# noisystreet/aither

Hardware: AMD Instinct MI355X
Metric: Mcell-updates/sec per iteration (residual+LU-SGS), 256^3 block; % HBM roofline (higher is better)
Workload: dtype f64

## Files before the change

### aither_amd/csrc/agx_api.hip

```cpp
#include "agx_kernels.hpp"
#include "agx_geometry.hpp"
#include "agx_mem.hpp"
#include "agx_switches.hpp"
#include <rccl/rccl.h>
#include <cstdarg>
#include <cstdio>
#include <cstring>
#include <cstdlib>
#include <cmath>
#include <vector>
#include <array>
#include <map>
#include <string>
#include <algorithm>
#include <memory>
#include <type_traits>

using namespace agx;

static char g_err[512] = "";
static int fail(const char* fmt, ...) {
  va_list ap;
  va_start(ap, fmt);
  vsnprintf(g_err, sizeof g_err, fmt, ap);
// ... 14 lines not shown
auto by_bool(bool v, F f) {
  return v ? f(std::true_type{}) : f(std::false_type{});
}
template <int V0, int... Vs, class F>
auto by_int(int v, F f) {
  if constexpr (sizeof...(Vs) == 0) return f(std::integral_constant<int, V0>{});
  else return v == V0 ? f(std::integral_constant<int, V0>{}) : by_int<Vs...>(v, f);
}

struct SweepGraphs {
  hipGraphExec_t g[2][2][2] = {};
  SweepGraphs() = default;
  SweepGraphs(SweepGraphs&& o) noexcept { memcpy(g, o.g, sizeof g); memset(o.g, 0, sizeof g); }
  ~SweepGraphs() { drop(); }
  hipGraphExec_t& at(bool forward, bool full, bool un_is_u) { return g[forward][full][un_is_u]; }
  void drop() {
    for (auto& g1 : g) for (auto& g2 : g1) for (auto& g3 : g2)
      if (g3) { hipGraphExecDestroy(g3); g3 = nullptr; }
  }
};

struct Block {
  BlockDev d;
  int global_pos = 0;
  DevBuf<double> slab;
  DevBuf<double> d2;
  DevBuf<double> blockmat;
  DevBuf<double> sweep_rec;
  bool sweep_geo_built = false;
  bool x_planes_current = false;
  bool x_is_zero = false;
  bool d2_state_current = false;
  bool resid_norms_current = false;
  DevBuf<double> mg_forcing, mg_mres, mg_xsave, mg_nodes;
  DevBuf<int> mg_tc, mg_start;
  DevBuf<double> mg_vf, mg_cf;
  const void *mg_tc_key = nullptr, *mg_vf_key = nullptr, *mg_cf_key = nullptr;
  bool node_built = false;
  DevBuf<double> nodes_dev, fcen;
  DevBuf<int> d2_tab;
  std::vector<int> dstart;
  SweepGraphs sweep_graph;
  DevBuf<int> kp_mem;
  unsigned kp_epoch = 0;
  long d2idx(int i, int j, int k) const {
    const int ie = i + d.ng, je = j + d.ng, de = ie + je;
    return (long)(k + d.ng) * d.d2.ps + dstart[de] + je - std::max(0, de - (d.d2.Pi - 1));
  }
  bool state_is_a = true;
  DevBuf<agx_bc_surface> surf_dev;
  std::vector<agx_bc_surface> surf_host;
  DevBuf<int> nr_off_dev;
  DevBuf<double> nr_mem;
  long nr_max = 0;
  DevBuf<int> wall_off_dev;
  DevBuf<WallVars> wall_mem;
  std::vector<WallSurfDev> wall_tab;
  DevBuf<WallSurfDev> wall_tab_dev;
  long wall_faces = 0;
  std::vector<LoadSurfDev> load_tab;
  DevBuf<LoadSurfDev> load_tab_dev;
  long load_faces = 0, load_chunks = 0;
  DevBuf<double> load_partial, load_fcen;
};

struct ConnSide {
// ... 94 lines not shown
  std::vector<std::pair<hipEvent_t, hipEvent_t>> ev_pool;
  std::vector<std::pair<int, int>> ev_used;
  double t_ms[G_NGROUP] = {};
  long t_n[G_NGROUP] = {};
};

static int my_side(const agx_ctx* c, const Conn& k);
static int implicit_begin(agx_ctx* c, int write_x);
static int halo_exchange_remote(agx_ctx* c, int what);
#if AGX_FAST
static int d2_prepare(agx_ctx* c, Block& blk, int write_x, int again, int norms);
#endif
namespace {
void resolve_timing(agx_ctx* c);
int lusgs_sweep(agx_ctx* c, Block& blk, bool forward, int full, hipStream_t st = nullptr);
}

namespace {
void x_changed(agx_ctx* c) {
  for (auto& blk : c->blocks) blk.x_planes_current = false;
}
void x_planes_copied(Block& b) { b.x_planes_current = true; }
void x_prepared(Block& b, bool left_zero) { b.x_is_zero = left_zero; }
void x_uploaded(Block& b) { b.x_is_zero = false; }
void x_swept(agx_ctx* c) {
  for (auto& blk : c->blocks) blk.x_is_zero = false;
}
void state_written(agx_ctx* c) {
  for (auto& blk : c->blocks) blk.d2_state_current = false;
}
void state_written(Block& b) { b.d2_state_current = false; }
void state_updated_d2(Block& b, bool wrote_d2) { b.d2_state_current = wrote_d2; }
void resid_written(agx_ctx* c) {
  for (auto& blk : c->blocks) blk.resid_norms_current = false;
}
void resid_norms_folded(Block& b) { b.resid_norms_current = true; }
void resid_norms_used(Block& b) { b.resid_norms_current = false; }
void planes_uploaded(Block& b) {
  b.d2_state_current = false;
  b.resid_norms_current = false;
}
void ghosts_filled_ahead(agx_ctx* c) { c->ghosts_prefilled = true; }
void ghost_fill_gone(agx_ctx* c) { c->ghosts_prefilled = false; }
void state_became_time_n(agx_ctx* c) {
  for (auto& blk : c->blocks)
    if (blk.nr_max > 0) c->ghosts_prefilled = false;
  c->state_is_time_n = true;
}
void state_left_time_n(agx_ctx* c) { c->state_is_time_n = false; }
void field_written_by_caller(agx_ctx* c) {
  ghost_fill_gone(c);
  state_left_time_n(c);
}


struct Timer {
  agx_ctx* c;
  int slot = -1;
  Timer(agx_ctx* ctx, int g) : c(ctx) {
    if (!c->timing) return;
    if (c->ev_used.size() >= 8192) resolve_timing(c);
    slot = (int)c->ev_used.size();
    if (slot >= (int)c->ev_pool.size()) {
      hipEvent_t a, b;
      if (hipEventCreate(&a) != hipSuccess || hipEventCreate(&b) != hipSuccess) {
        slot = -1;
        return;
      }
      c->ev_pool.emplace_back(a, b);
    }
    c->ev_used.emplace_back(g, slot);
    hipEventRecord(c->ev_pool[slot].first, c->stream);
  }
// ... 1718 lines not shown
    build_side_map(k.c, 1 - s, ng, idx_partner, idx_mine, ms);
    k.n_send = (long)ms.src.size();
    HIPCHK(k.send_src[space].upload(ms.src));
    *max_halo = std::max(*max_halo, (long)ms.src.size() * AGX_NEQ);
  }
  ConnSide& sd = k.side[s];
  sd.n = (long)m.dst.size();
  HIPCHK(sd.map[space].dst.upload(m.dst));
  if (partner_local) HIPCHK(sd.map[space].src.upload(m.src));
  *max_halo = std::max(*max_halo, (long)m.dst.size() * AGX_NEQ);
  if (space == 0) {
    sd.h_dst = std::move(m.dst);
    if (partner_local) sd.h_src = std::move(m.src);
  }
  return 0;
}
}

int agx_setup_finalize(agx_ctx* c) {
  HIPCHK(hipSetDevice(c->device));
  const int ng = c->cfg.n_ghost;
  if (!c->blocks.empty() && c->blocks[0].node_built && geo_complete(c)) return 1;
  long max_parts = 1, max_halo = 1;
  long march_parts = 0;
  for (auto& blk : c->blocks) {
    const dim3 g = cell_grid(blk.d, CELL_BLOCK);
    max_parts = std::max(max_parts, (long)g.x * g.y * g.z);
    march_parts += march_plan(c, blk.d).nparts;
    if (blk.d.d2.base) {
      max_parts = std::max(max_parts, mresid_wgs(c, blk.d));
#if AGX_FAST
      max_parts = std::max(max_parts, (long)((blk.d.d2.Pi + TT - 1) / TT) *
                                          ((blk.d.d2.Pj + TT - 1) / TT) * (blk.d.nk + 2 * blk.d.ng));
#endif
    }
  }
  max_parts = std::max(max_parts, march_parts);
  for (auto& k : c->conns) {
    const agx_connection& cc = k.c;
    const bool l0 = cc.rank[0] == c->rank, l1 = cc.rank[1] == c->rank;
    if (!l0 && !l1) continue;
    for (int s = 0; s < 2; ++s) {
      const bool mine = s == 0 ? l0 : l1, partner_mine = s == 0 ? l1 : l0;
      if (!mine) continue;
      const int lb = cc.local_block[s];
      if (lb < 0 || lb >= (int)c->blocks.size()) return fail("connection refers to unknown block");
      const Block* partner = partner_mine ? &c->blocks[cc.local_block[1 - s]] : nullptr;
      for (int space = 0; space < (use_d2(c) ? 2 : 1); ++space)
        if (halo_maps(k, s, space, ng, CellIndex{&c->blocks[lb], space},
                      CellIndex{partner, space}, partner_mine, &max_halo))
          return 1;
    }
  }
  if (halo_batch_plan(c, &max_halo)) return 1;
  if (ensure_halo_buf(c, 2 * max_halo)) return 1;
  std::vector<std::pair<int, int>> per_peer;
  for (size_t n = 0; n < c->conns.size(); ++n) {
    if (my_side(c, c->conns[n]) < 0) continue;
    agx_ctx::Remote r;
    r.cid = (int)n;
    r.count = (long)agx_halo_count(c, (int)n, AGX_HALO_STATE);
    const bool hb = c->have_ex && c->ex.host_buffers;
    const size_t cap = (size_t)std::max<long>(r.count, 1);
    HIPCHK(r.send.alloc(cap));
    HIPCHK(r.recv.alloc(cap));
    if (hb) {
// ... 580 lines not shown
                     cz->stream, bc.d, 0);
  const dim3 tb = CELL_BLOCK;
  hipLaunchKernelGGL(k_mg_nodes, dim3((bc.d.ni + tb.x) / tb.x, (bc.d.nj + tb.y) / tb.y, bc.d.nk + 1),
                     tb, 0, cz->stream, bc.d, bc.mg_nodes.get());
  HIPCHK(hipGetLastError());
  if (mg_order(cz, f)) return 1;
  hipLaunchKernelGGL(k_mg_prolong, cell_grid(bf.d, tb), tb, 0, f->stream, bf.d, m,
                     (const double*)bc.mg_nodes.get(), bc.d.ni, bc.d.nj, bc.d.nk);
  mg_x_records(cz, bc);
  mg_x_records(f, bf);
  if (mg_x_from_planes(cz, bc) || mg_x_from_planes(f, bf)) return 1;
  HIPCHK(hipGetLastError());
  return 0;
}

int agx_store_time_n(agx_ctx* c, int also_nm1) {
  if (flush_consn(c)) return 1;
  c->have_time_n = true;
  state_became_time_n(c);
  if (!c->no_lazy_consn && !also_nm1 && !c->use_gather && all_tile_ok(c)) { c->consn_pending = true; return 0; }
  for (auto& blk : c->blocks)
    hipLaunchKernelGGL(k_store_time_n, cell_grid(blk.d, CELL_BLOCK), CELL_BLOCK,
                       0, c->stream, blk.d, c->gas, also_nm1);
  HIPCHK(hipGetLastError());
  return 0;
}

int agx_phase_bc_faces(agx_ctx* c) {
  if (bc_faces(c)) return 1;
  c->ghost_fill_open = true;
  return 0;
}
int agx_phase_bc_edges(agx_ctx* c) { return bc_edges(c); }

int agx_phase_residual(agx_ctx* c, int mm, double cfl) {
  if (c->cfg.dt_nondim <= 0.0 && cfl <= 0.0)
    return fail("Neither dt or cfl was specified!");
  c->ghost_fill_open = false;
  c->sp.diag_add = c->mg_coarse ? 1 : 0;
  const bool fuse = can_fuse(c);
  resid_written(c);
  if (fuse) state_written(c);
  const int store_consn = !c->use_gather && all_tile_ok(c) && c->consn_pending && mm == 0;
  if (store_consn) c->consn_pending = false;
  else if (flush_consn(c)) return 1;
  {
    Timer t(c, G_RESID);
    long off = 0;
    for (auto& blk : c->blocks) {
      const MarchPlan mp = march_plan(c, blk.d);
      MarchArgs ma;
      memset(&ma, 0, sizeof ma);
      ma.kchunk = mp.kchunk;
      ma.mode = c->cfg.time_integration == AGX_TIME_RK4 ? 1 : 0;
      ma.store_consn = store_consn;
      const double rk_alpha[4] = {0.25, 1.0 / 3.0, 0.5, 1.0};
      ma.alpha = rk_alpha[mm & 3];
      ma.partials = c->partials.get() + off;
      ma.ablate = c->ablate;
      ma.plan = mp.tile;
      launch_inv(c, blk.d, cfl, fuse, ma, mp);
      off += mp.nparts;
      if (c->sp.implicit && c->sp.block) launch_block_diag(c, blk.d);
    }
  }
  HIPCHK(hipGetLastError());
// ... 32 lines not shown
        hipLaunchKernelGGL(k_rans_faces<0>, fgrid(1, 0, 0), tb, 0, c->stream, vb, c->gas, fourth, rec);
        hipLaunchKernelGGL(k_rans_faces<1>, fgrid(0, 1, 0), tb, 0, c->stream, vb, c->gas, fourth, rec);
        hipLaunchKernelGGL(k_rans_faces<2>, fgrid(0, 0, 1), tb, 0, c->stream, vb, c->gas, fourth, rec);
        hipLaunchKernelGGL(k_rans_cells, cell_grid(vb, tb), tb, 0, c->stream, vb, c->gas, c->sp,
                           cfl, fourth, rec);
      }
#else
    {
      const bool fourth = c->cfg.viscous_recon == AGX_VISC_RECON_CENTRAL_4TH;
      const bool wide_plane = (double)blk.d.nplane * 8.0 >= 4294967296.0;
      if (!AGX_FAST || c->visc_gather || ((fourth || c->sp.les) && (c->visc_march || wide_plane))) {
        hipLaunchKernelGGL(c->sp.les ? k_visc_residual_les : k_visc_residual,
                           cell_grid(blk.d, CELL_BLOCK), CELL_BLOCK, 0, c->stream, blk.d, c->gas,
                           c->sp, cfl, fourth ? 1 : 0);
      } else {
        const BlockDev& vb = blk.d;
        if (c->visc_march || wide_plane) {
          const int gx = (vb.ni + VTI - 1) / VTI, gy = (vb.nj + VTJ - 1) / VTJ;
          int nz = std::max(1, std::min(vb.nk / 8, (int)std::lround(2048.0 / (gx * gy))));
          const int kchunk = (vb.nk + nz - 1) / nz;
          nz = (vb.nk + kchunk - 1) / kchunk;
          hipLaunchKernelGGL(k_visc_march, dim3(gx, gy, nz), dim3(64, VTJ + 1), 0, c->stream,
                             vb, c->gas, c->sp, cfl, kchunk);
          continue;
        }
#if AGX_FAST
        const int gx = tile_count(vb.ni, fourth ? TILE_VISC_I_F4 : TILE_VISC_I);
        const int gy = tile_count(vb.nj, TILE_J);
        const long steps = (long)gx * gy * vb.nk;
        const int nwg = (int)std::min<long>(c->num_cu, std::max<long>(1, steps / 8));
        const TilePlan tp = tile_plan_of(c, gx, gy, vb.nk, nwg,
                                         fourth ? TILE_CHARGE_VISC_F4 : TILE_CHARGE_VISC,
                                         c->tile_order_visc);
        by_bool(c->sp.les != 0, [&](auto les) {
          by_bool(fourth, [&](auto f4) {
            hipLaunchKernelGGL((k_visc_tile<f4, decltype(les)::value>), dim3(nwg),
                               dim3(VT_L, VT_R), 0, c->stream, make_slab(vb), c->gas, c->sp, cfl,
                               gx, tp);
          });
        });
#endif
      }
    }
#endif
#if AGX_NEQ != 7
    if (c->sp.implicit && c->sp.block)
      for (auto& blk : c->blocks)
        hipLaunchKernelGGL(k_block_diag_visc, cell_grid(blk.d, CELL_BLOCK), CELL_BLOCK, 0,
                           c->stream, blk.d, c->gas, c->sp,
                           c->cfg.viscous_recon == AGX_VISC_RECON_CENTRAL_4TH ? 1 : 0);
#endif
    HIPCHK(hipGetLastError());
  }
  for (auto& blk : c->blocks)
    if (blk.nr_max > 0) {
      Timer t(c, G_BC);
      hipLaunchKernelGGL(k_nr_grads, dim3((blk.nr_max + 255) / 256, blk.d.nsurf), dim3(256), 0,
                         c->stream, blk.d, c->gas);
      HIPCHK(hipGetLastError());
    }
  return 0;
}

int agx_phase_explicit_update(agx_ctx* c, int mm, double* l2, agx_linf* linf) {
  const int mode = c->cfg.time_integration == AGX_TIME_RK4 ? 1 : 0;
  return update_pass(c, mode, mm, l2, linf);
}

#if AGX_FAST
static int d2_prepare(agx_ctx* c, Block& blk, int write_x, int again, int norms) {
  const BlockDev& b = blk.d;
  const dim3 grid((b.d2.Pi + TT - 1) / TT, (b.d2.Pj + TT - 1) / TT, b.nk + 2 * b.ng);
  const bool lean = blk.d2_state_current && !again;
  int ghost_s = 0;
  for (int q = 0; q < 6; ++q) ghost_s |= b.side_conn[q] != 0;
  const unsigned tag = write_x ? (unsigned)(++blk.kp_epoch) & 3u : 0u;
  by_bool(lean, [&](auto is_lean) {
    by_bool(norms != 0, [&](auto with_norms) {
      hipLaunchKernelGGL((k_lusgs_prepare<decltype(is_lean)::value, with_norms>), grid, dim3(256),
                         0, c->stream, b, c->gas, c->sp, write_x, tag, again, ghost_s,
                         c->partials.get());
    });
  });
  if (norms) {
    const size_t n = (size_t)(&blk - c->blocks.data());
    if (reduce_norms(c, n, (long)grid.x * grid.y * grid.z, c->norm_prepare() + n)) return 1;
    resid_norms_folded(blk);
  }
  return 0;
}
#endif
int agx_phase_implicit_begin(agx_ctx* c) { return implicit_begin(c, 1); }
static int implicit_begin(agx_ctx* c, int write_x) {
  x_changed(c);
  Timer t(c, G_PREPARE);
  c->sp.un_is_u = c->state_is_time_n ? 1 : 0;
  for (auto& blk : c->blocks) {
    const BlockDev& b = blk.d;
#if AGX_FAST
    if (b.d2.base) {
      bool conn = false;
      for (int q = 0; q < 6; ++q) conn = conn || b.side_conn[q] != 0;
      const int wx = write_x && (c->sp.requires_init || conn) ? 1 : 0;
      if (d2_prepare(c, blk, wx, 0, write_x && c->resid_norms_prepare ? 1 : 0)) return 1;
      x_prepared(blk, write_x && !wx);
      continue;
    }
#endif
    if (!c->sp.requires_init && write_x)
      hipLaunchKernelGGL(k_zero5, dim3((b.nplane + 255) / 256), dim3(256), 0,
                         c->stream, planes(b.x), b.nplane);
    hipLaunchKernelGGL(k_implicit_begin, cell_grid(b, CELL_BLOCK), CELL_BLOCK, 0,
                       c->stream, b, c->gas, c->sp, c->err_dev.get(), write_x);
    if (b.sw_geo) {
      hipLaunchKernelGGL(k_sweep_records, dim3((unsigned)((b.nplane + 255) / 256)), dim3(256), 0,
                         c->stream, b, c->sp, blk.sweep_geo_built ? 0 : 1);
      blk.sweep_geo_built = true;
    }
  }
  HIPCHK(hipGetLastError());
  return 0;
}

static void launch_dplur(agx_ctx* c, const BlockDev& b, int waits) {
  by_int<0, 1, 2>(solver_mode_of(c->sp), [&](auto mode) {
    hipLaunchKernelGGL(k_dplur<mode>, cell_grid(b, CELL_BLOCK), CELL_BLOCK, 0, c->stream, b,
                       c->gas, c->sp, waits);
  });
}

int agx_phase_relax_forward(agx_ctx* c, int sweep) {
  x_changed(c);
  x_swept(c);
  Timer t(c, G_SWEEP);
  const int full = sweep > 0 || c->sp.requires_init;
  if (is_lusgs_solver(c) && pipe_sweep_applicable(c)) return lusgs_sweep_pipe(c, true, full);
  if (is_lusgs_solver(c) && plane_sweep_all_applicable(c)) return lusgs_sweep_all(c, true, full);
// ... 438 lines not shown
```

### aither_amd/csrc/agx_kernels.hpp

```cpp
#pragma once
#include "agx_device.hpp"
#include "agx_lusgs.hpp"
#include "agx_tile_plan.hpp"

namespace agx {

struct BlockDev {
  int ni, nj, nk, ng;
  int ioff;
  long sx, sxy, nplane;
  int parent;
  double* state[AGX_NEQ];
  double* state2[AGX_NEQ];
  double* fa[3][4];
  double* vol;
  double* cen[3];
  double* wid[3];
  double* resid[AGX_NEQ];
  double* specrad;
  double* dt;
  double* consn[AGX_NEQ];
  double* consnm1[AGX_NEQ];
  double* x[AGX_NEQ];
  double* xold[AGX_NEQ];
// ... 60 lines not shown
  __device__ __forceinline__ double* snew(int e) const { return pl(sn + e); }
  __device__ __forceinline__ const double* wid(int d) const { return pl(PL_WID + d); }
  __device__ __forceinline__ const double* fa(int d, int c) const { return pl(PL_FA + 4 * d + c); }
  __device__ __forceinline__ long idx(int i, int j, int k) const {
    return (long)(k + ng) * sxy + (long)(j + ng) * sx + (i + ioff);
  }
  __device__ __forceinline__ void area(int d, long q, double* a) const {
#pragma unroll
    for (int c = 0; c < 4; ++c) a[c] = fa(d, c)[q];
  }
  __device__ __forceinline__ double ldb(int id, unsigned qb) const {
    return *reinterpret_cast<const double*>(reinterpret_cast<const char*>(pl(id)) + qb);
  }
  __device__ __forceinline__ void stb(int id, unsigned qb, double v) const {
    *reinterpret_cast<double*>(reinterpret_cast<char*>(pl(id)) + qb) = v;
  }
  __device__ __forceinline__ void areab(int d, unsigned qb, double* a) const {
#pragma unroll
    for (int c = 0; c < 4; ++c) a[c] = ldb(PL_FA + 4 * d + c, qb);
  }
};

struct SolverDev {
  double kappa, theta, zeta, relax, dual_time_cfl, dt_fixed, visc_cfl_coeff;
  int viscous, implicit, bdf2, requires_init, time_integration;
  int diag_add;
  int roe_jacobian;
  int un_is_u;
  int block;
  int les;
};
static_assert(sizeof(SolverDev) == 96, "SolverDev::les lies in the tail padding");

__device__ __forceinline__ void load5(double* const* p, long q, double* s) {
#pragma unroll
  for (int e = 0; e < AGX_NEQ; ++e) s[e] = p[e][q];
}
__device__ __forceinline__ void store5(double* const* p, long q, const double* s) {
#pragma unroll
  for (int e = 0; e < AGX_NEQ; ++e) p[e][q] = s[e];
}
__device__ __forceinline__ void load_area(const BlockDev& b, int d, long q, double* a) {
#pragma unroll
  for (int c = 0; c < 4; ++c) a[c] = b.fa[d][c][q];
}

template <int RECON, int LIM>
__device__ __forceinline__ void face_states_1d(double kappa, const double (*st)[AGX_NEQ],
                                               const double* w, int c, double* l, double* r) {
  if (RECON == AGX_RECON_CONSTANT) {
#pragma unroll
    for (int e = 0; e < AGX_NEQ; ++e) { l[e] = st[c - 1][e]; r[e] = st[c][e]; }
  } else if (RECON == AGX_RECON_MUSCL) {
    const double dPl = (w[c - 1] + w[c - 1]) / (w[c - 1] + w[c]);
    const double dMl = (w[c - 1] + w[c - 1]) / (w[c - 1] + w[c - 2]);
    const double dPr = (w[c] + w[c]) / (w[c] + w[c - 1]);
    const double dMr = (w[c] + w[c]) / (w[c] + w[c + 1]);
#pragma unroll
    for (int e = 0; e < AGX_NEQ; ++e) {
      l[e] = muscl<LIM>(st[c - 2][e], st[c - 1][e], st[c][e], dPl, dMl, kappa);
      r[e] = muscl<LIM>(st[c + 1][e], st[c][e], st[c - 1][e], dPr, dMr, kappa);
    }
  } else {
    const double cwl[5] = {w[c - 3], w[c - 2], w[c - 1], w[c], w[c + 1]};
    const double cwr[5] = {w[c + 2], w[c + 1], w[c], w[c - 1], w[c - 2]};
    WenoCoeffs kl, kr;
// ... 2036 lines not shown
  sh[threadIdx.x] = p;
  __syncthreads();
  for (int off = blockDim.x / 2; off > 0; off >>= 1) {
    if ((int)threadIdx.x < off) {
      NormPartial a = sh[threadIdx.x], o = sh[threadIdx.x + off];
      for (int e = 0; e < AGX_NEQ; ++e) a.l2[e] += o.l2[e];
      if (o.vmax > a.vmax || (o.vmax == a.vmax && o.lin < a.lin)) { a.vmax = o.vmax; a.lin = o.lin; }
      sh[threadIdx.x] = a;
    }
    __syncthreads();
  }
  if (threadIdx.x == 0) out[blockIdx.x] = sh[0];
}

__global__ void __launch_bounds__(256)
k_store_time_n(BlockDev b, GasDev g, int also_nm1) {
  const int i = blockIdx.x * blockDim.x + threadIdx.x;
  const int j = blockIdx.y * blockDim.y + threadIdx.y;
  const int k = blockIdx.z;
  if (i >= b.ni || j >= b.nj) return;
  const long q = b.idx(i, j, k);
  double s[AGX_NEQ], u[AGX_NEQ];
  load5(b.state, q, s);
  prim_to_cons(g, s, u);
  store5(b.consn, q, u);
  if (also_nm1) store5(b.consnm1, q, u);
}

__device__ __forceinline__ void rhs_b_r(const BlockDev& b, const GasDev& g,
                                        const SolverDev& sp, long q, const double* r,
                                        double* out) {
  const double thetaInv = 1.0 / sp.theta;
  if (sp.un_is_u && !sp.bdf2) {
#pragma unroll
    for (int e = 0; e < AGX_NEQ; ++e) out[e] = -thetaInv * r[e] - 0.0;
    return;
  }
  double s[AGX_NEQ], u[AGX_NEQ], un[AGX_NEQ];
  load5(b.state, q, s);
  load5(b.consn, q, un);
  prim_to_cons(g, s, u);
  const double vdt = b.vol[q] / (b.dt[q] * sp.theta);
  const double cN = vdt * (1.0 + sp.zeta);
#pragma unroll
  for (int e = 0; e < AGX_NEQ; ++e)
    out[e] = -thetaInv * r[e] - (sp.un_is_u ? 0.0 : cN * (u[e] - un[e]));
  if (sp.bdf2) {
    double um[AGX_NEQ];
    load5(b.consnm1, q, um);
    const double cM = vdt * sp.zeta;
#pragma unroll
    for (int e = 0; e < AGX_NEQ; ++e) out[e] += cM * (un[e] - um[e]);
  }
}
__device__ __forceinline__ void rhs_b(const BlockDev& b, const GasDev& g,
                                      const SolverDev& sp, long q, double* out) {
  double r[AGX_NEQ];
  load5(b.resid, q, r);
  rhs_b_r(b, g, sp, q, r, out);
}

__device__ __forceinline__ void rhs_bf_r(const BlockDev& b, const GasDev& g,
                                         const SolverDev& sp, long q, const double* r,
                                         double* out) {
  rhs_b_r(b, g, sp, q, r, out);
  if (b.mg_forcing) {
#pragma unroll
    for (int e = 0; e < AGX_NEQ; ++e) out[e] += b.mg_forcing[(long)e * b.nplane + q];
// ... 1440 lines not shown
```

### aither_amd/csrc/agx_lusgs.hpp

```cpp
#pragma once
#include "agx_device.hpp"

namespace agx {

enum {
  PA_S = 0,
  PA_B = 3,
  PA_X = 6,
  PA_F = 9,
  PA_COUNT = 15,
  D1_VF = 2 * PA_COUNT,
  D1_AD = D1_VF + 1,
  D2_DOUBLES = 2 * PA_COUNT + 4
};

struct D2Dev {
  double* base;
  long nd2, ps;
  const int* dstart;
  const int* ij_of_pos;
  int Pi, Pj;
  __device__ __forceinline__ double2* pa(int id) const {
    return reinterpret_cast<double2*>(base + 2L * id * nd2);
  }
  __device__ __forceinline__ double* vf() const { return base + (long)D1_VF * nd2; }
  __device__ __forceinline__ double* ad(int d) const { return base + (long)(D1_AD + d) * nd2; }
  __device__ __forceinline__ double ld_ad(int d, long cell) const { return ad(d)[cell]; }
  __device__ __forceinline__ double2 ld_pair(int id, long cell) const { return pa(id)[cell]; }
  __device__ __forceinline__ double ld_vf(long cell) const { return vf()[cell]; }
  __device__ __forceinline__ int jlo(int de) const { return max(0, de - (Pi - 1)); }
  __device__ __forceinline__ int pos2(int ie, int je) const {
    const int de = ie + je;
    return dstart[de] + je - jlo(de);
  }
};

struct KpBlk {
  double* base;
  const int* dstart;
  const agx_bc_surface* surf;
  long nd2, ps;
  int Pi, Pj, ni, nj, nk, ng;
  int nsurf, nsurf_i, nsurf_j, nsurf_k;
  int side_conn[6];
  __device__ __forceinline__ int dstart_cf(int de) const {
    const int a = min(Pi, Pj), bm = max(Pi, Pj);
    if (de <= a) return de * (de + 1) / 2;
    if (de <= bm) return a * (a + 1) / 2 + (de - a) * a;
    const int r = Pi + Pj - 1 - de;
    return Pi * Pj - r * (r + 1) / 2;
  }
  __device__ __forceinline__ const char* pab(int id) const {
    return reinterpret_cast<const char*>(base) + (size_t)id * (size_t)nd2 * 16;
  }
  __device__ __forceinline__ const char* vfb() const {
    return reinterpret_cast<const char*>(base) + (size_t)D1_VF * (size_t)nd2 * 8;
  }
  __device__ __forceinline__ const char* adb(int d) const {
    return reinterpret_cast<const char*>(base) + (size_t)(D1_AD + d) * (size_t)nd2 * 8;
  }
  __device__ __forceinline__ double ld_ad(int d, long cell) const {
    return *reinterpret_cast<const double*>(adb(d) + cell * 8);
  }
  __device__ __forceinline__ double2 ld_pair(int id, long cell) const {
    return *reinterpret_cast<const double2*>(pab(id) + cell * 16);
  }
  __device__ __forceinline__ double ld_vf(long cell) const {
    return *reinterpret_cast<const double*>(vfb() + cell * 8);
  }
  __device__ __forceinline__ int jlo(int de) const { return max(0, de - (Pi - 1)); }
};
struct KpGas { double hf, n, inv_n; };
__device__ __forceinline__ double2 ld16(const char* ubase, unsigned voff) {
  return *reinterpret_cast<const double2*>(ubase + voff);
}
__device__ __forceinline__ double ld8(const char* ubase, unsigned voff) {
  return *reinterpret_cast<const double*>(ubase + voff);
}

}
```

### aither_amd/csrc/agx_lusgs_kernels.hpp

```cpp
#pragma once

namespace agx {

constexpr int TT = 32;
constexpr int TRS = TT + 2;
__device__ __forceinline__ int tile_diag_index(int li, int lj) {
  const int dd = li + lj;
  if (dd < TT) return dd * (dd + 1) / 2 + lj;
  const int r = 2 * TT - 2 - dd;
  return TT * TT - (r + 1) * (r + 2) / 2 + (lj - (dd - (TT - 1)));
}
__device__ __forceinline__ void tile_table(unsigned short* s_tab) {
  const int tid = threadIdx.x;
#pragma unroll
  for (int m = 0; m < 4; ++m) {
    const int li = tid & (TT - 1), lj = (tid >> 5) + 8 * m;
    s_tab[tile_diag_index(li, lj)] = (unsigned short)(li | (lj << 8));
  }
}

__device__ __forceinline__ double kp_tagged(double v, unsigned tag) {
  const unsigned long long u = (unsigned long long)__double_as_longlong(v);
  return __longlong_as_double((long long)((u & ~3ull) | tag));
}
// ... 55 lines not shown
  __shared__ double sv[6][TT][TRS];
  __shared__ unsigned short s_tab[TT * TT];
  const D2Dev& z = b.d2;
  const int tid = threadIdx.x;
  tile_table(s_tab);
  const int i0 = blockIdx.x * TT, j0 = blockIdx.y * TT, ke = blockIdx.z;
  const int k = ke - b.ng;
  const int li = tid & (TT - 1);
  double bb[4][AGX_NEQ], x0[4][AGX_NEQ], ainv[4], vf[4];
  double l2[AGX_NEQ] = {0, 0, 0, 0, 0};
  double vmax = -1.0e300;
  long long vlin = 0x7fffffffffffffffLL;
#pragma unroll
  for (int m = 0; m < 4; ++m) {
    const int lj = (tid >> 5) + 8 * m;
    const int ie = i0 + li, je = j0 + lj;
    const int i = ie - b.ng, j = je - b.ng;
#pragma unroll
    for (int e = 0; e < AGX_NEQ; ++e) { bb[m][e] = 0.0; x0[m][e] = 0.0; }
    ainv[m] = 1.0;
    vf[m] = 0.0;
    double cs = 0.0;
    if (ie < z.Pi && je < z.Pj) {
      const long q = b.idx(i, j, k);
      const bool phys = i >= 0 && i < b.ni && j >= 0 && j < b.nj && k >= 0 && k < b.nk;
      if (!LEAN || (ghost_s && !phys)) {
        double s[AGX_NEQ];
#pragma unroll
        for (int e = 0; e < AGX_NEQ; ++e) { s[e] = b.state[e][q]; sv[e][lj][li] = s[e]; }
        if (s[0] > 0.0) cs = sound_speed(g, s);
        if (sp.viscous) vf[m] = cell_visc_factor(g, s);
      }
      if (phys) {
        double dvt = (b.vol[q] * (1.0 + sp.zeta)) / (b.dt[q] * sp.theta);
        if (sp.dual_time_cfl > 0.0) dvt += fmax(b.specrad[q], 0.0) / sp.dual_time_cfl;
        const double a = again ? b.ainv[q] : b.a[q] * sp.relax + dvt;
        b.ainv[q] = a;
        if (sp.diag_add) b.a[q] = a;
        ainv[m] = 1.0 / a;
        double r[AGX_NEQ];
        load5(b.resid, q, r);
        rhs_bf_r(b, g, sp, q, r, bb[m]);
        if (NORMS) {
          const long lin0 = (((long)k * b.nj + j) * b.ni + i) * AGX_NEQ;
#pragma unroll
          for (int e = 0; e < AGX_NEQ; ++e) {
            l2[e] += r[e] * r[e];
            if (r[e] > vmax || (r[e] == vmax && lin0 + e < vlin)) { vmax = r[e]; vlin = lin0 + e; }
          }
        }
        if (sp.requires_init) {
#pragma unroll
          for (int e = 0; e < AGX_NEQ; ++e) x0[m][e] = bb[m][e] * ainv[m];
        }
      }
    }
    sv[5][lj][li] = cs;
  }
  __syncthreads();
  long pos[4];
  int tli[4], tlj[4];
  bool st_s[4];
#pragma unroll
  for (int m = 0; m < 4; ++m) {
    const unsigned tl = s_tab[tid + 256 * m];
    tli[m] = tl & 0xff; tlj[m] = tl >> 8;
    const int ie = i0 + tli[m], je = j0 + tlj[m];
    pos[m] = -1;
    st_s[m] = !LEAN;
// ... 672 lines not shown
```

### aither_amd/csrc/agx_visc_tile.hpp

```cpp
#pragma once
#include "agx_tile_plan.hpp"

namespace agx {

constexpr int VT_L = 64, VT_R = 8;
constexpr int VT_OI = VT_L - 2, VT_OJ = VT_R - 2;
static_assert(VT_OI == TILE_VISC_I && VT_L - 4 == TILE_VISC_I_F4 && VT_OJ == TILE_J,
              "the plan's tile sizes (agx_tile_plan.hpp) are this kernel's");
enum { VS_S0 = 0, VS_SM = 4, VS_SP = 8, VS_AI0 = 12, VS_AJ0 = 15, VS_AJ1 = 18, VS_AK0 = 21,
       VS_AK1 = 24, VS_VOL = 27, VS_WJ = 28, VS_RHO = 29, VS_MU = 30, VS_AI1 = 31, VS_WI = 34,
       VS_FJ = 35, VS_COUNT = 39 };

#ifndef VT_LDSAREA
#define VT_LDSAREA 1
#endif
#ifndef VT_EDGE_BARRIER
#define VT_EDGE_BARRIER __builtin_amdgcn_sched_barrier(0)
#endif
struct VRef { int var, row, lane; };
using VShared = double (*)[VT_L][VS_COUNT];
__device__ __forceinline__ void vt_ld4(VShared sh, const VRef& r, double* o) {
#pragma unroll
  for (int c = 0; c < 4; ++c) o[c] = sh[r.row][r.lane][r.var + c];
}
// ... 102 lines not shown
    tf = pf * fast_rcp(rf);
    mu = g.scaling * c4(c0[5], mL_, mU_, c3[5]);
  } else {
    const double iw = fast_rcp(wL + wU);
    const double cD = wU * iw, cU = wL * iw;
#pragma unroll
    for (int c = 0; c < 3; ++c) vf[c] = cD * vU[c] + cU * vL[c];
    const double rf = cD * rU_ + cU * rL_;
    tf = (cD * rU_ * vU[3] + cU * rL_ * vL[3]) * fast_rcp(rf);
    mu = g.scaling * (cD * mU_ + cU * mL_);
  }
  if constexpr (LES) {
    f[4] = wale_eddy_visc(grad, 0.5 * (wL + wU));
    mu += g.scaling * f[4];
  }
  const double lambda = -(2.0 / 3.0) * mu;
  const double trace = grad[0][0] + grad[1][1] + grad[2][2];
  double tau[3];
#pragma unroll
  for (int r = 0; r < 3; ++r) {
    const double mm = (grad[r][0] + grad[0][r]) * aF[0] + (grad[r][1] + grad[1][r]) * aF[1] +
                      (grad[r][2] + grad[2][r]) * aF[2];
    tau[r] = lambda * trace * aF[r] + mu * mm;
  }
  double kk = conductivity(g, tf) * g.scaling;
  if constexpr (LES) kk += g.scaling * f[4] * g.cp / g.turb_prandtl;
  const double tg = grad[0][3] * aF[0] + grad[1][3] * aF[1] + grad[2][3] * aF[2];
  f[0] = tau[0];
  f[1] = tau[1];
  f[2] = tau[2];
  f[3] = dot3(tau, vf) + kk * tg;
}

template <bool F4, bool LES = false>
__global__ void __launch_bounds__(VT_L * VT_R)
k_visc_tile(SlabDev b, GasDev g, SolverDev sp, double cfl, int gx, TilePlan tp) {
  __shared__ double sh[VT_R][VT_L][VS_COUNT];
  constexpr int NF = LES ? 5 : 4;
  constexpr int LO = F4 ? 2 : 1;
  constexpr int OI = F4 ? VT_L - 4 : VT_OI;
  const int l = threadIdx.x, ty = threadIdx.y;
  TileWalk walk = tile_walk_begin(tp);
  TileSeg seg;
  while (tile_walk_next(tp, walk, seg)) {
  const int col = seg.col, k0 = seg.k0, k1 = seg.k1;
  const int ci = (col % gx) * OI - LO + l, cj = (col / gx) * VT_OJ - 1 + ty;
  const bool inner = l >= LO && l < LO + OI && ty >= 1 && ty <= VT_OJ;
  const bool own = inner && ci < b.ni && cj < b.nj;
  const bool do_i = l >= LO && l <= LO + OI && ty >= 1 && ty <= VT_OJ && ci <= b.ni && cj < b.nj;
  const bool do_j = ty >= 1 && l >= LO && l < LO + OI && cj <= b.nj && ci < b.ni;
  const int ic = min(ci, F4 ? b.ni + 1 : b.ni), jc = min(cj, F4 ? b.nj + 1 : b.nj);
  const unsigned qc = (unsigned)(b.idx(ic, jc, 0) * 8);
  const unsigned sk = (unsigned)(b.sxy * 8), sj = (unsigned)(b.sx * 8);
  const int kcmax = b.nk + b.ng - 1, kfmax = b.nk + b.ng;
  auto ld_state = [&](int k, double* s4, double& rho, double& mu) {
    const unsigned q = qc + (unsigned)min(k, kcmax) * sk;
    rho = b.ldb(b.st + 0, q);
    s4[0] = b.ldb(b.st + 1, q); s4[1] = b.ldb(b.st + 2, q); s4[2] = b.ldb(b.st + 3, q);
    s4[3] = rho > 0.0 ? b.ldb(b.st + 4, q) * fast_rcp(rho * g.R) : 0.0;
    mu = rho > 0.0 ? viscosity(g, s4[3]) : 0.0;
  };
  auto rq_state = [&](int k, double* raw) {
    const unsigned q = qc + (unsigned)min(k, kcmax) * sk;
#pragma unroll
    for (int e = 0; e < 5; ++e) raw[e] = b.ldb(b.st + e, q);
  };
  auto cv_state = [&](const double* raw, double* s4, double& rho, double& mu) {
    rho = raw[0];
    s4[0] = raw[1]; s4[1] = raw[2]; s4[2] = raw[3];
    s4[3] = rho > 0.0 ? raw[4] * fast_rcp(rho * g.R) : 0.0;
    mu = rho > 0.0 ? viscosity(g, s4[3]) : 0.0;
  };
  auto ld_avec = [&](int d, unsigned q, double* a3) {
    const double mag = b.ldb(PL_FA + 4 * d + 3, q);
    a3[0] = b.ldb(PL_FA + 4 * d + 0, q) * mag; a3[1] = b.ldb(PL_FA + 4 * d + 1, q) * mag;
    a3[2] = b.ldb(PL_FA + 4 * d + 2, q) * mag;
  };
  auto rq_avec = [&](int d, unsigned q, double* raw) {
#pragma unroll
    for (int c = 0; c < 4; ++c) raw[c] = b.ldb(PL_FA + 4 * d + c, q);
  };
  auto cv_avec = [&](const double* raw, double* a3) {
    a3[0] = raw[0] * raw[3]; a3[1] = raw[1] * raw[3]; a3[2] = raw[2] * raw[3];
  };
  auto PUT4 = [&](int var, const double* v) {
#pragma unroll
    for (int c = 0; c < 4; ++c) sh[ty][l][var + c] = v[c];
// ... 136 lines not shown
#pragma unroll
        for (int c = 0; c < 4; ++c) c3[c] = S2[c];
        c3[4] = R2; c3[5] = MU2; w3 = WK2;
      };
      vt_face<F4, LES>(sh, g, me0, meP, meR, meR, R1, MU1, true, SPr, aF, aFm, AK2, iu, il, ju, jl, V0,
                  V1, WK0, WK1, fk_up, wide);
    }
    __builtin_amdgcn_sched_barrier(0);
    double nRaw[5], rAI[4], rAJ[4], rAK[4], rAIp[4] = {0, 0, 0, 0}, rAJp[4] = {0, 0, 0, 0};
    const unsigned qn = qc + (unsigned)(kk + 1) * sk;
    const unsigned qn2 = qc + (unsigned)min(kk + 2, kcmax) * sk;
    rq_state(F4 ? kk + 3 : kk + 2, nRaw);
    rq_avec(0, qn2, rAI);
    rq_avec(1, qn2, rAJ);
    rq_avec(2, qc + (unsigned)min(kk + 3, kfmax) * sk, rAK);
    if (mem_i) rq_avec(0, qn + 8, rAIp);
    if (mem_j) rq_avec(1, qn + sj, rAJp);
    const double nV = b.ldb(PL_VOL, qn2);
    const double nWK = b.ldb(PL_WID + 2, F4 ? qc + (unsigned)min(kk + 3, kcmax) * sk : qn2);
    double nEJ[6] = {0, 0, 0, 0, 0, 0}, nEw = 0;
    if (ej_row) {
      const unsigned qe = qej + (unsigned)(kk + 1) * sk;
#pragma unroll
      for (int e = 0; e < 5; ++e) nEJ[e] = b.ldb(b.st + e, qe);
      nEw = b.ldb(PL_WID + 1, qe);
    }
    const double nwi = b.ldb(PL_WID + 0, qn), nwj = b.ldb(PL_WID + 1, qn);
    __syncthreads();
    if (own && !pre) {
      const unsigned q = qc + (unsigned)kk * sk;
      double res[AGX_NEQ];
#pragma unroll
      for (int e = 1; e < AGX_NEQ; ++e) res[e] = b.ldb(PL_RESID + e, q);
#pragma unroll
      for (int c = 0; c < 4; ++c)
        res[1 + c] += ((racc[c] - sh[ty + 1][l][VS_FJ + c]) + fk_lo[c]) - fk_up[c];
      const double ivol = fast_rcp(V0);
      const double vfac = visc_max_term(g, R0) * visc_term(g, MU0);
      double sr = b.ldb(PL_SPECRAD, q);
      double diag = sp.implicit ? b.ldb(PL_A, q) : 0.0;
      double ai0[3], aj0[3], ak0[3], ak1[3];
      LD3(VS_AI0, ty, l, ai0); LD3(VS_AJ0, ty, l, aj0);
      LD3(VS_AK0, ty, l, ak0); LD3(VS_AK1, ty, l, ak1);
      const double fm[3] = {0.5 * (fast_sqrt(dot3(ai0, ai0)) + fast_sqrt(dot3(AIp, AIp))),
                            0.5 * (fast_sqrt(dot3(aj0, aj0)) + fast_sqrt(dot3(AJp, AJp))),
                            0.5 * (fast_sqrt(dot3(ak0, ak0)) + fast_sqrt(dot3(ak1, ak1)))};
      if constexpr (LES) {
        const double mut_lo[3] = {fi[4], fj[4], fk_lo[4]};
        const double vmax = visc_max_term(g, R0);
#pragma unroll
        for (int d = 0; d < 3; ++d) {
          const double vterm = g.scaling * (MU0 * g.inv_prandtl + mut_lo[d] / g.turb_prandtl);
          const double vsr = vmax * vterm * fm[d] * fm[d] * ivol;
          sr += vsr * sp.visc_cfl_coeff;
          diag += 2.0 * vsr;
        }
        const double sixth = 1.0 / 6.0;
        double ev = sixth * fi[4];
        ev += sixth * mut_iup;
        ev += sixth * fj[4];
        ev += sixth * sh[ty + 1][l][VS_MU];
        ev += sixth * fk_lo[4];
        ev += sixth * fk_up[4];
        b.stb(PL_EDDY_LES, q, ev);
      } else {
#pragma unroll
      for (int d = 0; d < 3; ++d) {
        const double vsr = vfac * fm[d] * fm[d] * ivol;
        sr += vsr * sp.visc_cfl_coeff;
        diag += 2.0 * vsr;
      }
      }
#pragma unroll
      for (int e = 1; e < AGX_NEQ; ++e) b.stb(PL_RESID + e, q, res[e]);
      b.stb(PL_SPECRAD, q, sr);
      if (sp.implicit) b.stb(PL_A, q, diag);
      b.stb(PL_DT, q, sp.dt_fixed > 0.0 ? sp.dt_fixed : cfl * (V0 * fast_rcp(fmax(sr, 0.0))));
    }
    {
      double t3[3], t4[4];
      double nS[4], nR, nMU, nAI[3], nAJ[3], nAK[3], nAIp[3], nAJp[3];
      cv_state(nRaw, nS, nR, nMU);
      cv_avec(rAI, nAI); cv_avec(rAJ, nAJ); cv_avec(rAK, nAK);
      cv_avec(rAIp, nAIp); cv_avec(rAJp, nAJp);
      LD4(VS_S0, ty, l, t4); PUT4(VS_SM, t4);
      LD4(VS_SP, ty, l, t4); PUT4(VS_S0, t4);
      if (F4) {
        PUT4(VS_SP, S2);
        RM = sh[ty][l][VS_RHO];
        sh[ty][l][VS_RHO] = R1; R1 = R2; R2 = nR;
        if constexpr (LES) { MUM = MU0r; MU0r = MU1; }
        else { MUM = sh[ty][l][VS_MU]; sh[ty][l][VS_MU] = MU1; }
        MU1 = MU2; MU2 = nMU;
#pragma unroll
        for (int c = 0; c < 4; ++c) S2[c] = nS[c];
        if (ej_row) {
          const double rho = nEJ[0];
          EJ[0] = nEJ[1]; EJ[1] = nEJ[2]; EJ[2] = nEJ[3];
          EJ[3] = rho > 0.0 ? nEJ[4] * fast_rcp(rho * g.R) : 0.0;
          EJ[4] = rho;
          EJ[5] = rho > 0.0 ? viscosity(g, EJ[3]) : 0.0;
          EJ[6] = nEw;
        }
      } else {
        PUT4(VS_SP, nS);
        sh[ty][l][VS_RHO] = R1; R1 = nR;
        if constexpr (LES) MU0r = MU1;
        else sh[ty][l][VS_MU] = MU1;
        MU1 = nMU;
      }
      LD3(VS_AI1, ty, l, t3); PUT3(VS_AI0, t3); PUT3(VS_AI1, nAI);
      LD3(VS_AJ1, ty, l, t3); PUT3(VS_AJ0, t3); PUT3(VS_AJ1, nAJ);
      LD3(VS_AK1, ty, l, t3); PUT3(VS_AK0, t3); PUT3(VS_AK1, AK2);
      sh[ty][l][VS_VOL] = V1; V1 = nV;
      sh[ty][l][VS_WI] = nwi; sh[ty][l][VS_WJ] = nwj;
      if (F4) { WKM = WK0; WK0 = WK1; WK1 = WK2; WK2 = nWK; }
      else { WK0 = WK1; WK1 = nWK; }
#pragma unroll
      for (int c = 0; c < NF; ++c) fk_lo[c] = fk_up[c];
#pragma unroll
      for (int c = 0; c < 3; ++c) { AK2[c] = nAK[c]; AIp[c] = nAIp[c]; AJp[c] = nAJp[c]; }
    }
  }
  __syncthreads();
  }
}

}
```

Measured before the change: 1524.

## Fuse LU-SGS RHS preparation and residual norms into viscous tile kernel

When the block meets a set of simple conditions (central, no LES, no connections, time-n state, no multigrid forcing), the viscous tile kernel now also computes the LU-SGS diagonal, writes the scaled RHS and inverse diagonal into the d2 plane layout, and accumulates per-wavefront residual norm partials. The separate d2_prepare pass and its timer are skipped for such blocks, which removes a full re-read of residual, dt and volume arrays. The cost is extra registers and stores in an already heavy kernel, and more state flags that must stay consistent.

```diff
diff --git a/aither_amd/csrc/agx_api.hip b/aither_amd/csrc/agx_api.hip
--- a/aither_amd/csrc/agx_api.hip
+++ b/aither_amd/csrc/agx_api.hip
@@ -70,6 +70,7 @@
   bool x_is_zero = false;
   bool d2_state_current = false;
   bool resid_norms_current = false;
+  bool rhs_in_d2 = false;
   DevBuf<double> mg_forcing, mg_mres, mg_xsave, mg_nodes;
   DevBuf<int> mg_tc, mg_start;
   DevBuf<double> mg_vf, mg_cf;
@@ -230,13 +231,16 @@
 void state_written(Block& b) { b.d2_state_current = false; }
 void state_updated_d2(Block& b, bool wrote_d2) { b.d2_state_current = wrote_d2; }
 void resid_written(agx_ctx* c) {
-  for (auto& blk : c->blocks) blk.resid_norms_current = false;
+  for (auto& blk : c->blocks) blk.resid_norms_current = blk.rhs_in_d2 = false;
 }
 void resid_norms_folded(Block& b) { b.resid_norms_current = true; }
 void resid_norms_used(Block& b) { b.resid_norms_current = false; }
+void rhs_written_by_residual(Block& b) { b.rhs_in_d2 = true; }
+void rhs_taken(Block& b) { b.rhs_in_d2 = false; }
 void planes_uploaded(Block& b) {
   b.d2_state_current = false;
   b.resid_norms_current = false;
+  b.rhs_in_d2 = false;
 }
 void ghosts_filled_ahead(agx_ctx* c) { c->ghosts_prefilled = true; }
 void ghost_fill_gone(agx_ctx* c) { c->ghosts_prefilled = false; }
@@ -2021,6 +2025,7 @@
 #if AGX_FAST
       max_parts = std::max(max_parts, (long)((blk.d.d2.Pi + TT - 1) / TT) *
                                           ((blk.d.d2.Pj + TT - 1) / TT) * (blk.d.nk + 2 * blk.d.ng));
+      max_parts = std::max(max_parts, (long)c->num_cu * VT_R);
 #endif
     }
   }
@@ -2667,6 +2672,18 @@
   return 0;
 }
 int agx_phase_bc_edges(agx_ctx* c) { return bc_edges(c); }
+
+#if AGX_FAST
+static bool rhs_form_applies(const agx_ctx* c, const Block& blk) {
+  const BlockDev& b = blk.d;
+  bool conn = false;
+  for (int q = 0; q < 6; ++q) conn = conn || b.side_conn[q] != 0;
+  return b.d2.base && blk.d2_state_current && c->d2_state_update &&
+         c->resid_norms_prepare && !conn && !c->sp.requires_init && c->state_is_time_n &&
+         !c->sp.bdf2 && !b.mg_forcing && !c->sp.diag_add && !c->mg_coarse &&
+         !(c->sp.dual_time_cfl > 0.0) && !c->sp.les;
+}
+#endif
 
 int agx_phase_residual(agx_ctx* c, int mm, double cfl) {
   if (c->cfg.dt_nondim <= 0.0 && cfl <= 0.0)
@@ -2765,11 +2782,35 @@
         const TilePlan tp = tile_plan_of(c, gx, gy, vb.nk, nwg,
                                          fourth ? TILE_CHARGE_VISC_F4 : TILE_CHARGE_VISC,
                                          c->tile_order_visc);
+        if (!fourth && rhs_form_applies(c, blk)) {
+          if (c->in_iterate) {
+            c->sp.un_is_u = 1;
+            VtRhs<VT_RHS_FULL> rz;
+            rz.partials = c->partials.get();
+            rz.pab = reinterpret_cast<char*>(vb.d2.base + 2L * PA_B * vb.d2.nd2);
+            rz.arr16 = vb.d2.nd2 * 16;
+            rz.ps16 = vb.d2.ps * 16;
+            rz.Pi = vb.d2.Pi;
+            rz.Pj = vb.d2.Pj;
+            hipLaunchKernelGGL((k_visc_tile<false, false, VT_RHS_FULL>), dim3(nwg),
+                               dim3(VT_L, VT_R), 0, c->stream, make_slab(vb), c->gas, c->sp, cfl,
+                               gx, tp, rz);
+            rhs_written_by_residual(blk);
+          } else {
+            hipLaunchKernelGGL((k_visc_tile<false, false, VT_RHS_NORMS>), dim3(nwg),
+                               dim3(VT_L, VT_R), 0, c->stream, make_slab(vb), c->gas, c->sp, cfl,
+                               gx, tp, VtRhs<VT_RHS_NORMS>{c->partials.get()});
+          }
+          const size_t n = (size_t)(&blk - c->blocks.data());
+          if (reduce_norms(c, n, (long)nwg * VT_R, c->norm_prepare() + n)) return 1;
+          resid_norms_folded(blk);
+          continue;
+        }
         by_bool(c->sp.les != 0, [&](auto les) {
           by_bool(fourth, [&](auto f4) {
             hipLaunchKernelGGL((k_visc_tile<f4, decltype(les)::value>), dim3(nwg),
                                dim3(VT_L, VT_R), 0, c->stream, make_slab(vb), c->gas, c->sp, cfl,
-                               gx, tp);
+                               gx, tp, VtRhs<VT_RHS_NONE>{});
           });
         });
 #endif
@@ -2826,16 +2867,27 @@
 int agx_phase_implicit_begin(agx_ctx* c) { return implicit_begin(c, 1); }
 static int implicit_begin(agx_ctx* c, int write_x) {
   x_changed(c);
-  Timer t(c, G_PREPARE);
+  bool any_pass = false;
+  for (auto& blk : c->blocks) any_pass = any_pass || !(write_x && blk.rhs_in_d2);
+  std::unique_ptr<Timer> t;
+  if (any_pass) t = std::make_unique<Timer>(c, G_PREPARE);
   c->sp.un_is_u = c->state_is_time_n ? 1 : 0;
   for (auto& blk : c->blocks) {
     const BlockDev& b = blk.d;
 #if AGX_FAST
+    const bool rhs_done = write_x && blk.rhs_in_d2;
+    rhs_taken(blk);
+    if (rhs_done) {
+      x_prepared(blk, true);
+      resid_norms_folded(blk);
+      continue;
+    }
     if (b.d2.base) {
       bool conn = false;
       for (int q = 0; q < 6; ++q) conn = conn || b.side_conn[q] != 0;
       const int wx = write_x && (c->sp.requires_init || conn) ? 1 : 0;
-      if (d2_prepare(c, blk, wx, 0, write_x && c->resid_norms_prepare ? 1 : 0)) return 1;
+      const int norms = write_x && c->resid_norms_prepare && !blk.resid_norms_current ? 1 : 0;
+      if (d2_prepare(c, blk, wx, 0, norms)) return 1;
       x_prepared(blk, write_x && !wx);
       continue;
     }
diff --git a/aither_amd/csrc/agx_kernels.hpp b/aither_amd/csrc/agx_kernels.hpp
--- a/aither_amd/csrc/agx_kernels.hpp
+++ b/aither_amd/csrc/agx_kernels.hpp
@@ -116,6 +116,19 @@
 };
 static_assert(sizeof(SolverDev) == 96, "SolverDev::les lies in the tail padding");
 
+__device__ __forceinline__ void lusgs_b_time_n(const SolverDev& sp, const double* r,
+                                               double* out) {
+  const double thetaInv = 1.0 / sp.theta;
+#pragma unroll
+  for (int e = 0; e < AGX_NEQ; ++e) out[e] = -thetaInv * r[e] - 0.0;
+}
+__device__ __forceinline__ double lusgs_dvt(const SolverDev& sp, double vol, double dt) {
+  return (vol * (1.0 + sp.zeta)) / (dt * sp.theta);
+}
+__device__ __forceinline__ double lusgs_diag(const SolverDev& sp, double a, double dvt) {
+  return a * sp.relax + dvt;
+}
+
 __device__ __forceinline__ void load5(double* const* p, long q, double* s) {
 #pragma unroll
   for (int e = 0; e < AGX_NEQ; ++e) s[e] = p[e][q];
@@ -2218,8 +2231,7 @@
                                         double* out) {
   const double thetaInv = 1.0 / sp.theta;
   if (sp.un_is_u && !sp.bdf2) {
-#pragma unroll
-    for (int e = 0; e < AGX_NEQ; ++e) out[e] = -thetaInv * r[e] - 0.0;
+    lusgs_b_time_n(sp, r, out);
     return;
   }
   double s[AGX_NEQ], u[AGX_NEQ], un[AGX_NEQ];
diff --git a/aither_amd/csrc/agx_lusgs.hpp b/aither_amd/csrc/agx_lusgs.hpp
--- a/aither_amd/csrc/agx_lusgs.hpp
+++ b/aither_amd/csrc/agx_lusgs.hpp
@@ -35,6 +35,14 @@
   }
 };
 
+__device__ __forceinline__ int d2_dstart_cf(int Pi, int Pj, int de) {
+  const int a = min(Pi, Pj), bm = max(Pi, Pj);
+  if (de <= a) return de * (de + 1) / 2;
+  if (de <= bm) return a * (a + 1) / 2 + (de - a) * a;
+  const int r = Pi + Pj - 1 - de;
+  return Pi * Pj - r * (r + 1) / 2;
+}
+
 struct KpBlk {
   double* base;
   const int* dstart;
@@ -43,13 +51,7 @@
   int Pi, Pj, ni, nj, nk, ng;
   int nsurf, nsurf_i, nsurf_j, nsurf_k;
   int side_conn[6];
-  __device__ __forceinline__ int dstart_cf(int de) const {
-    const int a = min(Pi, Pj), bm = max(Pi, Pj);
-    if (de <= a) return de * (de + 1) / 2;
-    if (de <= bm) return a * (a + 1) / 2 + (de - a) * a;
-    const int r = Pi + Pj - 1 - de;
-    return Pi * Pj - r * (r + 1) / 2;
-  }
+  __device__ __forceinline__ int dstart_cf(int de) const { return d2_dstart_cf(Pi, Pj, de); }
   __device__ __forceinline__ const char* pab(int id) const {
     return reinterpret_cast<const char*>(base) + (size_t)id * (size_t)nd2 * 16;
   }
diff --git a/aither_amd/csrc/agx_lusgs_kernels.hpp b/aither_amd/csrc/agx_lusgs_kernels.hpp
--- a/aither_amd/csrc/agx_lusgs_kernels.hpp
+++ b/aither_amd/csrc/agx_lusgs_kernels.hpp
@@ -111,9 +111,9 @@
         if (sp.viscous) vf[m] = cell_visc_factor(g, s);
       }
       if (phys) {
-        double dvt = (b.vol[q] * (1.0 + sp.zeta)) / (b.dt[q] * sp.theta);
+        double dvt = lusgs_dvt(sp, b.vol[q], b.dt[q]);
         if (sp.dual_time_cfl > 0.0) dvt += fmax(b.specrad[q], 0.0) / sp.dual_time_cfl;
-        const double a = again ? b.ainv[q] : b.a[q] * sp.relax + dvt;
+        const double a = again ? b.ainv[q] : lusgs_diag(sp, b.a[q], dvt);
         b.ainv[q] = a;
         if (sp.diag_add) b.a[q] = a;
         ainv[m] = 1.0 / a;
diff --git a/aither_amd/csrc/agx_visc_tile.hpp b/aither_amd/csrc/agx_visc_tile.hpp
--- a/aither_amd/csrc/agx_visc_tile.hpp
+++ b/aither_amd/csrc/agx_visc_tile.hpp
@@ -158,10 +158,27 @@
   f[3] = dot3(tau, vf) + kk * tg;
 }
 
-template <bool F4, bool LES = false>
+enum { VT_RHS_NONE = 0, VT_RHS_NORMS = 1, VT_RHS_FULL = 2 };
+template <int RHS>
+struct VtRhs {};
+template <>
+struct VtRhs<VT_RHS_NORMS> {
+  NormPartial* partials;
+};
+template <>
+struct VtRhs<VT_RHS_FULL> {
+  NormPartial* partials;
+  char* pab;
+  long arr16, ps16;
+  int Pi, Pj;
+};
+template <bool F4, bool LES = false, int RHS = VT_RHS_NONE>
 __global__ void __launch_bounds__(VT_L * VT_R)
-k_visc_tile(SlabDev b, GasDev g, SolverDev sp, double cfl, int gx, TilePlan tp) {
+k_visc_tile(SlabDev b, GasDev g, SolverDev sp, double cfl, int gx, TilePlan tp, VtRhs<RHS> rz) {
+  static_assert(!RHS || (!F4 && !LES), "the RHS forms exist for `central` without LES");
   __shared__ double sh[VT_R][VT_L][VS_COUNT];
+  double nl2[AGX_NEQ] = {0, 0, 0, 0, 0}, nvmax = -1.0e300;
+  long long nvlin = 0x7fffffffffffffffLL;
   constexpr int NF = LES ? 5 : 4;
   constexpr int LO = F4 ? 2 : 1;
   constexpr int OI = F4 ? VT_L - 4 : VT_OI;
@@ -179,6 +196,13 @@
   const unsigned qc = (unsigned)(b.idx(ic, jc, 0) * 8);
   const unsigned sk = (unsigned)(b.sxy * 8), sj = (unsigned)(b.sx * 8);
   const int kcmax = b.nk + b.ng - 1, kfmax = b.nk + b.ng;
+  unsigned pd2 = 0;
+  long long lin_c = 0;
+  if constexpr (RHS == VT_RHS_FULL) {
+    const int ie = ic + b.ng, je = jc + b.ng, de = ie + je;
+    pd2 = (unsigned)(d2_dstart_cf(rz.Pi, rz.Pj, de) + je - max(0, de - (rz.Pi - 1))) * 16u;
+  }
+  if constexpr (RHS != VT_RHS_NONE) lin_c = ((long long)jc * b.ni + ic) * AGX_NEQ;
   auto ld_state = [&](int k, double* s4, double& rho, double& mu) {
     const unsigned q = qc + (unsigned)min(k, kcmax) * sk;
     rho = b.ldb(b.st + 0, q);
@@ -381,6 +405,7 @@
       double res[AGX_NEQ];
 #pragma unroll
       for (int e = 1; e < AGX_NEQ; ++e) res[e] = b.ldb(PL_RESID + e, q);
+      if constexpr (RHS != VT_RHS_NONE) res[0] = b.ldb(PL_RESID + 0, q);
 #pragma unroll
       for (int c = 0; c < 4; ++c)
         res[1 + c] += ((racc[c] - sh[ty + 1][l][VS_FJ + c]) + fk_lo[c]) - fk_up[c];
@@ -424,7 +449,30 @@
       for (int e = 1; e < AGX_NEQ; ++e) b.stb(PL_RESID + e, q, res[e]);
       b.stb(PL_SPECRAD, q, sr);
       if (sp.implicit) b.stb(PL_A, q, diag);
-      b.stb(PL_DT, q, sp.dt_fixed > 0.0 ? sp.dt_fixed : cfl * (V0 * fast_rcp(fmax(sr, 0.0))));
+      const double dt = sp.dt_fixed > 0.0 ? sp.dt_fixed : cfl * (V0 * fast_rcp(fmax(sr, 0.0)));
+      b.stb(PL_DT, q, dt);
+      if constexpr (RHS == VT_RHS_FULL) {
+        const double a = lusgs_diag(sp, diag, lusgs_dvt(sp, V0, dt));
+        b.stb(PL_AINV, q, a);
+        const double ia = 1.0 / a;
+        double bb[AGX_NEQ];
+        lusgs_b_time_n(sp, res, bb);
+        char* pb = rz.pab + (long)(kk + b.ng) * rz.ps16 + pd2;
+        *reinterpret_cast<double2*>(pb) = make_double2(bb[0], bb[1]);
+        *reinterpret_cast<double2*>(pb + rz.arr16) = make_double2(bb[2], bb[3]);
+        *reinterpret_cast<double2*>(pb + 2 * rz.arr16) = make_double2(bb[4], ia);
+      }
+      if constexpr (RHS != VT_RHS_NONE) {
+        const long long lin0 = lin_c + (long long)kk * ((long long)b.nj * b.ni * AGX_NEQ);
+#pragma unroll
+        for (int e = 0; e < AGX_NEQ; ++e) {
+          nl2[e] += res[e] * res[e];
+          if (res[e] > nvmax || (res[e] == nvmax && lin0 + e < nvlin)) {
+            nvmax = res[e];
+            nvlin = lin0 + e;
+          }
+        }
+      }
     }
     {
       double t3[3], t4[4];
@@ -473,6 +521,23 @@
   }
   __syncthreads();
   }
+  if constexpr (RHS != VT_RHS_NONE) {
+    for (int off = 32; off > 0; off >>= 1) {
+#pragma unroll
+      for (int e = 0; e < AGX_NEQ; ++e) nl2[e] += __shfl_down(nl2[e], off, 64);
+      const double ov = __shfl_down(nvmax, off, 64);
+      const long long ol = __shfl_down(nvlin, off, 64);
+      if (ov > nvmax || (ov == nvmax && ol < nvlin)) { nvmax = ov; nvlin = ol; }
+    }
+    if (threadIdx.x == 0) {
+      NormPartial p;
+#pragma unroll
+      for (int e = 0; e < AGX_NEQ; ++e) p.l2[e] = nl2[e];
+      p.vmax = nvmax;
+      p.lin = nvlin;
+      rz.partials[(long)blockIdx.x * VT_R + threadIdx.y] = p;
+    }
+  }
 }
 
 }
```

After: 1595 (median of 6 runs). 4.7% higher.
